# thenoobychocobo/gpt2-image-captioning

Measured on AMD Instinct MI355X. Metric: training images/sec + greedy captions/sec, GPT2-small+CLIP-B/32 at 1/2/4/8 GPU, higher is better.
Workload: dtype bf16

## Files before the change

gpt2-image-captioning_amd/csrc/gemm.hip:

```cpp
#include <cstdlib>

#include "gemm_tile.h"
#include "gemm_launch.h"

namespace icap {

template <typename TI>
__device__ __forceinline__ uint4 ln_chunk(const uint4 a, float mean, float rs, const float* g, const float* bt);
template <>
__device__ __forceinline__ uint4 ln_chunk<bf16_t>(const uint4 a, float mean, float rs, const float* g, const float* bt) {
  const uint32_t w[4] = {a.x, a.y, a.z, a.w};
  uint32_t o[4];
#pragma unroll
  for (int q = 0; q < 4; ++q) {
    const float v0 = (__uint_as_float(w[q] << 16) - mean) * rs * g[2 * q] + bt[2 * q];
    const float v1 = (__uint_as_float(w[q] & 0xffff0000u) - mean) * rs * g[2 * q + 1] + bt[2 * q + 1];
    o[q] = f2bf2(v0, v1);
  }
  return make_uint4(o[0], o[1], o[2], o[3]);
}
template <>
__device__ __forceinline__ uint4 ln_chunk<float>(const uint4 a, float mean, float rs, const float* g, const float* bt) {
  return make_uint4(__float_as_uint((__uint_as_float(a.x) - mean) * rs * g[0] + bt[0]),
                    __float_as_uint((__uint_as_float(a.y) - mean) * rs * g[1] + bt[1]),
// ... 359 lines not shown

static int gemm_acquire() { return diag_env("ICAP_FUSED_ACQUIRE", 0) == 1 ? 1 : 0; }
static int gemm_diag() { return diag_env("ICAP_GEMM_DIAG", 0) & 3; }

typedef int (*TileLauncher)(const GemmPlan&, const icap_gemm_args&, int, hipStream_t);
static TileLauncher tile_launcher(const GemmPlan& pl, const icap_gemm_args& p) {
  switch (pl.variant) {
    case V_ROLES_KOUT: return launch_tile_roles_kout;
    case V_ROLES: return launch_tile_roles;
    case V_ROLES160: return launch_tile_roles160;
    case V_ROLES96: return launch_tile_roles96;
    case V_ROLES192: return launch_tile_roles192;
    case V_R256: return launch_tile_r256;
    case V_W192: case V_W192_RING: return launch_tile_w192;
    case V_KOUT_DB: case V_KOUT_S3: return launch_tile_kout;
    case V_DB: case V_S3: case V_S4: case V_N12: case V_N13: case V_RING:
      if (pl.actk >= ACT_LNS) return launch_tile_ln;
      if (pl.actk >= ACT_FWD) return launch_tile_act;
      return p.in_dtype == ICAP_BF16 ? launch_tile_bf16 : p.in_dtype == ICAP_FP8_MX ? launch_tile_mx : launch_tile_f32;
  }
  return nullptr;
}

extern "C" const char* icap_gemm_kernel_name(const icap_gemm_args* a) {
  if (a == nullptr) return nullptr;
  GemmPlan pl;
  if (gemm_plan(*a, pl, device_cus(), plan_diag()) != ICAP_OK) return nullptr;
  return gemm_plan_kernel_name(*a, pl);
}

extern "C" int icap_gemm_plan_info(const icap_gemm_args* a, int32_t* splits, int32_t* fused) {
  ICAP_REQUIRE(a != nullptr && splits != nullptr && fused != nullptr, "icap_gemm_plan_info: null pointer");
  GemmPlan pl;
  const int rc = gemm_plan(*a, pl, device_cus(), plan_diag());
  if (rc != ICAP_OK) return rc;
  *splits = pl.skinny || pl.g256 || pl.g8p ? 1 : pl.splits;
  *fused = pl.fused ? 1 : 0;
  return ICAP_OK;
}

static bool group_force128() {
  const char* e = std::getenv("ICAP_GROUP128");
  return e != nullptr && std::atoi(e) == 1;
}

extern "C" int icap_gemm_group(const icap_gemm_args* a, int32_t n, void* stream) {
  ICAP_REQUIRE(a != nullptr && n >= 1 && n <= ICAP_GEMM_GROUP_MAX, "icap_gemm_group: 1 ... 8 products");
  static_assert(ICAP_GEMM_GROUP_MAX == GROUP_MAX, "the group's planner and its kernel argument hold the same count");
  GemmGroup g;
  g.n = 0;
  g.swap = 0;
  g.tstart[0] = 0;
  int64_t Ms[ICAP_GEMM_GROUP_MAX], Ns[ICAP_GEMM_GROUP_MAX];
  for (int i = 0; i < n; ++i) {
    const icap_gemm_args& p = a[i];
    icap_gemm_args q = p;
    q.split_k = 1;
    q.path = 0;
    if (const int rc = gemm_validate(q); rc != ICAP_OK) return rc;
    ICAP_REQUIRE(p.trans_ab && p.in_dtype == ICAP_BF16 && p.c_dtype == ICAP_F32,
                 "icap_gemm_group: K-outer (trans_ab) bf16 products with an fp32 C");
    ICAP_REQUIRE(p.act == ICAP_ACT_NONE && p.dact == ICAP_ACT_NONE && !p.bias && !p.resid && !p.aux && !p.ln_gamma &&
                     !p.ln_wsum && !p.ln_stats_in && !p.ln_stats_out && p.drop_p == 0.f && !p.m_dev,
                 "icap_gemm_group: plain products only (alpha, beta; no epilogue operands)");
    if (p.M == 0 || p.N == 0) continue;
    ICAP_REQUIRE(p.K > 0, "icap_gemm_group: K must be positive");
    const int k = g.n;
    g.a[k] = p;
    g.a[k].split_k = 1;
    g.a[k].tickets = nullptr;
    g.nk[k] = (int)((p.K + 63) / 64) | (gemm_diag() << 28);
    Ms[k] = p.M, Ns[k] = p.N;
    ++g.n;
  }
  if (g.n == 0) return ICAP_OK;
  const int cus = (int)device_cus();
  const GroupPlan gp = gemm_group_plan(Ms, Ns, g.n, cus, group_force128());
  ICAP_REQUIRE(gp.total < (1ll << 30), "icap_gemm_group: too many tiles");
  for (int k = 0; k < g.n; ++k) {
    if (gp.big && ((gp.swap >> k) & 1)) {
      icap_gemm_args& p = g.a[k];
      std::swap(p.A, p.B);
      std::swap(p.lda, p.ldb);
      std::swap(p.M, p.N);
    }
    g.tiles_n[k] = gp.tiles_n[k];
    g.tstart[k + 1] = g.tstart[k] + gp.tiles_m[k] * gp.tiles_n[k];
  }
  g.swap = gp.big ? gp.swap : 0u;
  launch_group_kout(g, cus, gp.big, reinterpret_cast<hipStream_t>(stream));
  return check_launch("icap_gemm_group");
}

extern "C" int icap_gemm(const icap_gemm_args* a, void* stream) {
  ICAP_REQUIRE(a != nullptr, "icap_gemm: null args");
  if (a->M == 0 || a->N == 0) return ICAP_OK;
  GemmPlan pl;
  const int prc = gemm_plan(*a, pl, device_cus(), plan_diag());
  if (prc != ICAP_OK) return prc;
  icap_gemm_args pk = *a;
  if (!pl.fused) pk.tickets = nullptr;
  const icap_gemm_args& p = pk;
  hipStream_t s = reinterpret_cast<hipStream_t>(stream);
  const uint32_t thr = pl.thr;
  const float inv_keep = pl.inv_keep;
  if (pl.skinny) {
    const dim3 sgrid(pl.grid_x, pl.grid_y), sblock(pl.block_x);
#define ICAP_SK(TI, TC, NT, U) hipLaunchKernelGGL((gemm_skinny_kernel<TI, TC, NT, 2, U>), sgrid, sblock, 0, s, p, thr, inv_keep)
#define ICAP_SKINNY_BF(TC)                                                                 \
  switch (pl.nt * 100 + pl.sku) {                                                          \
    case 103: ICAP_SK(bf16_t, TC, 1, 3); break;                                            \
    case 104: ICAP_SK(bf16_t, TC, 1, 4); break;                                            \
    case 106: ICAP_SK(bf16_t, TC, 1, 6); break;                                            \
    case 112: ICAP_SK(bf16_t, TC, 1, 12); break;                                           \
    case 203: ICAP_SK(bf16_t, TC, 2, 3); break;                                            \
    case 204: ICAP_SK(bf16_t, TC, 2, 4); break;                                            \
    case 206: ICAP_SK(bf16_t, TC, 2, 6); break;                                            \
    case 303: ICAP_SK(bf16_t, TC, 3, 3); break;                                            \
    case 304: ICAP_SK(bf16_t, TC, 3, 4); break;                                            \
    case 306: ICAP_SK(bf16_t, TC, 3, 6); break;                                            \
    case 403: ICAP_SK(bf16_t, TC, 4, 3); break;                                            \
    case 404: ICAP_SK(bf16_t, TC, 4, 4); break;                                            \
    default: ICAP_SK(bf16_t, TC, 4, 6); break;                                             \
  }
#define ICAP_SKINNY_F32(TC)                                                                \
  switch (pl.nt) {                                                                         \
    case 1: ICAP_SK(float, TC, 1, 6); break;                                               \
    case 2: ICAP_SK(float, TC, 2, 6); break;                                               \
    case 3: ICAP_SK(float, TC, 3, 6); break;                                               \
    default: ICAP_SK(float, TC, 4, 6); break;                                              \
  }
    if (p.in_dtype == ICAP_BF16) {
      if (p.c_dtype == ICAP_BF16) { ICAP_SKINNY_BF(bf16_t) } else { ICAP_SKINNY_BF(float) }
    } else {
      if (p.c_dtype == ICAP_BF16) { ICAP_SKINNY_F32(bf16_t) } else { ICAP_SKINNY_F32(float) }
    }
#undef ICAP_SKINNY_BF
#undef ICAP_SKINNY_F32
#undef ICAP_SK
    return check_launch("icap_gemm(skinny)");
  }
  if (pl.g256) return gemm256_launch(p, thr, inv_keep, s);
  if (pl.g8p) return gemm8p_launch(pl, p, s);
  const int sp = pl.splits;
  const int skew = gemm_plan_skew(p, pl, plan_diag());
  const int nks = pl.nk_split | (skew << 20) | (gemm_diag() << 28) | (gemm_acquire() << 30);
  const dim3 rgrid((unsigned)((p.M * (p.N / 4) + 255) / 256));
  const TileLauncher launch = tile_launcher(pl, p);
  if (launch == nullptr) return gemm_no_instantiation(pl);
  if (const int rc = launch(pl, p, nks, s); rc != ICAP_OK) return rc;
  if (sp > 1 && !pl.fused) {
    if (p.c_dtype == ICAP_BF16)
      hipLaunchKernelGGL((gemm_splitk_reduce<bf16_t>), rgrid, dim3(256), 0, s, p, sp, thr, inv_keep);
    else
      hipLaunchKernelGGL((gemm_splitk_reduce<float>), rgrid, dim3(256), 0, s, p, sp, thr, inv_keep);
  }
  return check_launch("icap_gemm");
}
```

gpt2-image-captioning_amd/csrc/gemm256.hip:

```cpp
#include "gemm_common.h"

namespace icap {
namespace g256 {
constexpr int BM = 256, BN = 256;
constexpr int HT = 128 * GROWB;
constexpr int TB = 4 * HT;
constexpr int ELD = 68;
constexpr int EW = 64 * ELD * 4;
constexpr int SMEM = (2 * TB > 8 * EW) ? 2 * TB : 8 * EW;
typedef uint32_t u32x4_t __attribute__((ext_vector_type(4)));
}

#define G256_RD(dst, addr, off) asm volatile("ds_read_b128 %0, %1 offset:" #off : "=v"(dst) : "v"(addr))

template <typename TC>
__global__ __launch_bounds__(512, 1) void gemm256_kernel(icap_gemm_args p, int tiles_n, uint32_t drop_thresh,
                                                        float inv_keep) {
  using namespace g256;
  __shared__ __attribute__((aligned(16))) char smem[SMEM];
  const int tid = threadIdx.x, lane = tid & 63;
  const int wave = __builtin_amdgcn_readfirstlane(tid >> 6);
  const int wr = wave >> 2, wc = wave & 3;
  const int fr = lane & 15, fg = lane >> 4;
  const int G = gridDim.x, bid = blockIdx.x;
  const int xcd = bid & 7, q8 = G >> 3, r8 = G & 7;
  const int wg = (xcd < r8 ? xcd * (q8 + 1) : r8 * (q8 + 1) + (xcd - r8) * q8) + (bid >> 3);
  const int tm = wg / tiles_n, tn = wg - tm * tiles_n;
  const int64_t M = p.M, N = p.N, K = p.K;
  const int64_t m0 = (int64_t)tm * BM, n0 = (int64_t)tn * BN;
  const int64_t mr = M - m0 < BM ? M - m0 : BM, nr = N - n0 < BN ? N - n0 : BN;
  const int nk = (int)((K + 63) / 64);
  const bf16_t* Ag = reinterpret_cast<const bf16_t*>(p.A);
  const bf16_t* Bg = reinterpret_cast<const bf16_t*>(p.B);
  const __amdgpu_buffer_rsrc_t ra = make_rsrc_u(Ag + m0 * p.lda, (uint64_t)((mr - 1) * p.lda + K) * 2);
  const __amdgpu_buffer_rsrc_t rb = make_rsrc_u(Bg + n0 * p.ldb, (uint64_t)((nr - 1) * p.ldb + K) * 2);

  const int c = (lane & 7) ^ (lane >> 3);
  uint32_t voff[4][2];
#pragma unroll
  for (int h = 0; h < 4; ++h)
#pragma unroll
    for (int i = 0; i < 2; ++i) {
      const int lr = (i * 8 + wave) * 8 + (lane >> 3);
      int trow;
      if (h == 0) trow = (lr & 63) + (lr >> 6) * 128;
      else if (h == 3) trow = (lr & 63) + (lr >> 6) * 128 + 64;
      else if (h == 1) trow = (lr >> 5) * 64 + (lr & 31);
      else trow = (lr >> 5) * 64 + 32 + (lr & 31);
      const int64_t ld = (h == 0 || h == 3) ? p.lda : p.ldb;
      voff[h][i] = (uint32_t)((trow * ld + c * 8) * 2);
// ... 183 lines not shown
```

gpt2-image-captioning_amd/csrc/gemm8p.hip:

```cpp
#include <utility>

#include "gemm_common.h"
#include "gemm_plan.h"

namespace icap {
namespace g8p {
constexpr int BM = 256;
constexpr int HTA = 128 * GROWB;
typedef uint32_t u32x4_t __attribute__((ext_vector_type(4)));
template <int BN>
struct Geo {
  static constexpr int WCN = BN / 4;
  static constexpr int QN = WCN / 2;
  static constexpr int NJ = QN / 16;
  static constexpr int HTB = (BN / 2) * GROWB;
  static constexpr int TB = 2 * HTA + 2 * HTB;
  static constexpr int BPW = BN / 128;
  static constexpr int ELD = WCN + 4;
  static constexpr int EW = 64 * ELD * 4;
  static constexpr int NBUF = BN == 128 ? 3 : 2;
  static constexpr int SMEM = (NBUF * TB > 8 * EW) ? NBUF * TB : 8 * EW;
  static constexpr int LPR = WCN / 8;
  static constexpr int RPI = 64 / LPR;
};
}

// ... 9 lines not shown

#define G8P_RD(dst, addr, off) asm volatile("ds_read_b128 %0, %1 offset:" #off : "=v"(dst) : "v"(addr))

template <typename TC, int BN, int ACT>
__global__ __launch_bounds__(512, 1) void gemm8p_kernel(icap_gemm_args p, int tiles_n, uint32_t drop_thresh,
                                                       float inv_keep) {
  using namespace g8p;
  using G = Geo<BN>;
  constexpr int AK = ACT & 0xFF;
  constexpr int LNX = ACT >> 8;
  constexpr int NJ = G::NJ, WCN = G::WCN, QN = G::QN, BPW = G::BPW, TB = G::TB, HTB = G::HTB, NBUF = G::NBUF;
  constexpr int LA = NBUF - 1;
  __shared__ __attribute__((aligned(16))) char smem[G::SMEM + (LNX == 2 ? 8 * BM : 0)];
  const int tid = threadIdx.x, lane = tid & 63;
  const int wave = __builtin_amdgcn_readfirstlane(tid >> 6);
  const int wr = wave >> 2, wc = wave & 3;
  const int fr = lane & 15, fg = lane >> 4;
  const int64_t M = p.M, N = p.N, K = p.K;
  const int64_t Mv = p.m_dev && (int64_t)*p.m_dev < M ? (int64_t)*p.m_dev : M;
  const int bid = blockIdx.x;
  const int tiles_mv = (int)((Mv + BM - 1) / BM);
  const int nwg = tiles_mv * tiles_n;
  if (bid >= nwg) return;
  const int xcd = bid & 7, q8 = nwg >> 3, r8 = nwg & 7;
  const int wg = (xcd < r8 ? xcd * (q8 + 1) : r8 * (q8 + 1) + (xcd - r8) * q8) + (bid >> 3);
  const int tm = wg / tiles_n, tn = wg - tm * tiles_n;
  const int64_t m0 = (int64_t)tm * BM, n0 = (int64_t)tn * BN;
  G8P_STAMP(1);
  const int64_t mr = Mv - m0 < BM ? Mv - m0 : BM, nr = N - n0 < BN ? N - n0 : BN;
  const int nk = (int)((K + 63) / 64);
  const bf16_t* Ag = reinterpret_cast<const bf16_t*>(p.A);
  const bf16_t* Bg = reinterpret_cast<const bf16_t*>(p.B);
  const __amdgpu_buffer_rsrc_t ra = make_rsrc_u(Ag + m0 * p.lda, (uint64_t)((mr - 1) * p.lda + K) * 2);
  const __amdgpu_buffer_rsrc_t rb = make_rsrc_u(Bg + n0 * p.ldb, (uint64_t)((nr - 1) * p.ldb + K) * 2);

  const int c = (lane & 7) ^ (lane >> 3);
  uint32_t voa[2][2], vob[2][BPW];
#pragma unroll
  for (int i = 0; i < 2; ++i) {
    const int lr = (i * 8 + wave) * 8 + (lane >> 3);
    const int trow = (lr & 63) + (lr >> 6) * 128;
    voa[0][i] = (uint32_t)((trow * p.lda + c * 8) * 2);
    voa[1][i] = (uint32_t)(((trow + 64) * p.lda + c * 8) * 2);
  }
#pragma unroll
  for (int i = 0; i < BPW; ++i) {
    const int lr = (i * 8 + wave) * 8 + (lane >> 3);
    const int trow = (lr / QN) * WCN + (lr % QN);
    vob[0][i] = (uint32_t)((trow * p.ldb + c * 8) * 2);
// ... 294 lines not shown
```

gpt2-image-captioning_amd/csrc/gemm_plan.cpp:

```cpp
#include "gemm_plan.h"

#include <cstdio>

namespace icap {

PlanDiag plan_diag() {
  PlanDiag d;
  d.var_heavy = diag_env("ICAP_VAR_HEAVY", d.var_heavy);
  d.var_act = diag_env("ICAP_VAR_ACT", d.var_act);
  d.var_light = diag_env("ICAP_VAR_LIGHT", d.var_light);
  d.fused_s = diag_env("ICAP_FUSED_S", d.fused_s);
  d.fused_nst = diag_env("ICAP_FUSED_NST", d.fused_nst);
  if (const int v = diag_env("ICAP_FUSED_MINK", 0); v >= 2) d.fused_mink = v;
  d.kskew = diag_env("ICAP_KSKEW", d.kskew);
  d.kout_fused = diag_env("ICAP_KOUT_FUSED", 0) == 1;
  d.spec_act = diag_env("ICAP_SPEC_ACT", 1) != 0;
  d.force_tile = diag_env("ICAP_FORCE_TILE", d.force_tile);
  d.w192r = diag_env("ICAP_W192R", d.w192r);
  return d;
}

static bool al16(const void* ptr) { return (reinterpret_cast<uintptr_t>(ptr) & 15) == 0; }
static int64_t cdiv(int64_t a, int64_t b) { return (a + b - 1) / b; }
static bool plain(const icap_gemm_args& p) { return p.act == ICAP_ACT_NONE && p.dact == ICAP_ACT_NONE; }

int gemm_validate(const icap_gemm_args& p) {
  ICAP_REQUIRE(p.M >= 0 && p.N >= 0 && p.K >= 0, "icap_gemm: negative size");
  ICAP_REQUIRE(p.path == 0 || p.path == 1 || (p.path >= 3 && p.path <= 12), "icap_gemm: path must be 0, 1 or 3 ... 12");
  ICAP_REQUIRE(p.A && p.B && p.C, "icap_gemm: null operand");
  ICAP_REQUIRE(p.in_dtype == ICAP_F32 || p.in_dtype == ICAP_BF16 || p.in_dtype == ICAP_FP8_MX,
               "icap_gemm: bad in_dtype");
  ICAP_REQUIRE(p.c_dtype == ICAP_F32 || p.c_dtype == ICAP_BF16, "icap_gemm: bad c_dtype");
  const bool mx = p.in_dtype == ICAP_FP8_MX;
  if (mx) {
    ICAP_REQUIRE(p.K % 128 == 0 && p.lda % 16 == 0 && p.ldb % 16 == 0,
                 "icap_gemm: FP8_MX needs K % 128 == 0 and lda, ldb multiples of 16");
    ICAP_REQUIRE(p.a_scale && p.b_scale && al16(p.a_scale) && al16(p.b_scale),
                 "icap_gemm: FP8_MX needs 16-byte aligned a_scale / b_scale");
    ICAP_REQUIRE(!p.trans_ab && !p.ln_gamma && p.path != 3, "icap_gemm: FP8_MX takes no trans_ab / ln / path 3");
    ICAP_REQUIRE((p.K / 32) * ((p.M + 63) / 64) * 64 < 0x7fffffffll && (p.K / 32) * ((p.N + 63) / 64) * 64 < 0x7fffffffll,
                 "icap_gemm: FP8_MX scale arrays must stay below 2 GiB");
// ... 332 lines not shown
    pl.nk_split = (int)c.nk;
    return ICAP_OK;
  }
  int rc;
  if ((rc = plan_skinny(c, pl)) != PASS) return rc;
  if ((rc = plan_g256(c, pl)) != PASS) return rc;
  if ((rc = plan_g8p(c, pl)) != PASS) return rc;
  if ((rc = plan_roles_kout(c, pl)) != PASS) return rc;
  TileSplit ts;
  if ((rc = plan_tile_split(c, ts)) != ICAP_OK) return rc;
  if ((rc = plan_roles(c, pl)) != PASS) return rc;
  if ((rc = plan_r256(c, ts, pl)) != PASS) return rc;
  if ((rc = plan_w192(c, ts, pl)) != PASS) return rc;
  return plan_tile128(c, ts, pl);
}

int gemm_plan_skew(const icap_gemm_args& p, const GemmPlan& pl, const PlanDiag& diag) {
  const TileVariantInfo* t = tile_variant(pl.variant);
  if (t == nullptr || t->natural_k()) return 0;
  if (p.path == 1 || p.path >= 6 || p.in_dtype == ICAP_FP8_MX || pl.nk_split > 64) return 0;
  return diag.kskew > 0 && diag.kskew < 256 ? diag.kskew : 0;
}

const char* gemm_plan_kernel_name(const icap_gemm_args& a, const GemmPlan& pl) {
  static thread_local char buf[160];
  const char* ti = a.in_dtype == ICAP_BF16 ? "unsigned short" : a.in_dtype == ICAP_FP8_MX ? "icap::fp8_t" : "float";
  const char* tc = a.c_dtype == ICAP_BF16 ? "unsigned short" : "float";
  if (pl.g256) {
    snprintf(buf, sizeof buf, "icap::gemm256_kernel<%s>", tc);
  } else if (pl.g8p) {
    snprintf(buf, sizeof buf, "icap::gemm8p_kernel<%s, %d, %d>", tc, pl.g8p, pl.actk);
  } else if (pl.skinny) {
    snprintf(buf, sizeof buf, "icap::gemm_skinny_kernel<%s, %s, %d, 2, %d>", ti, tc, pl.nt, pl.sku);
  } else if (const TileVariantInfo* t = tile_variant(pl.variant)) {
    snprintf(buf, sizeof buf, "icap::gemm_kernel<%s, %s, %d, %d, %d, %d, %d, %d, %s, %d%s>", ti, tc, t->nst, t->minb, t->wm,
             t->wn, t->tm, t->tn, t->kout ? "true" : "false", pl.actk, t->roles ? ", true" : "");
  } else {
    return nullptr;
  }
  return buf;
}

int gemm_no_instantiation(const GemmPlan& pl) {
  set_error("icap_gemm: no instantiation of " + (pl.g8p ? "the 8-phase kernel of width " + std::to_string(pl.g8p)
                                                         : "tile variant " + std::to_string(pl.variant)) +
            " with epilogue kind " + std::to_string(pl.actk) + " for these dtypes");
// ... 23 lines not shown
```

gpt2-image-captioning_amd/csrc/gemm_plan.h:

```cpp
#pragma once
#include "gemm_consts.h"
#include "host_common.h"

namespace icap {


struct EpiCaps {
  unsigned fwd = 0, bwd = 0;
  bool ln_producer = false;
  bool ln_consumer = false;
  unsigned ln_fwd = 0;
  bool ln_any = false;
  bool f32_c_plain = true;
};
constexpr unsigned A_(int act) { return 1u << act; }
constexpr unsigned A_GN = A_(ICAP_ACT_GELU_NEW), A_QG = A_(ICAP_ACT_QUICK_GELU), A_RELU = A_(ICAP_ACT_RELU),
                   A_ERF = A_(ICAP_ACT_GELU_ERF);
constexpr unsigned IN_F32 = 1u << ICAP_F32, IN_BF16 = 1u << ICAP_BF16, IN_MX = 1u << ICAP_FP8_MX;

enum TileVariant : int {
  V_DB = 0,
  V_S3 = 4,
  V_S4 = 5,
  V_N12 = 12,
// ... 82 lines not shown
  bool g256 = false;
  int g8p = 0;
  int nt = 1;
  int sku = 3;
  int variant = V_DB;
  int splits = 1, nk_split = 0, tiles_n = 0;
  bool fused = false;
  int actk = ACT_ANY;
  unsigned grid_x = 1, grid_y = 1, block_x = 1;
  uint32_t thr = 0;
  float inv_keep = 1.f;
};

struct PlanDiag {
  int var_heavy = V_S3, var_act = V_S3, var_light = V_S3;
  int fused_s = 0;
  int fused_nst = 0;
  int fused_mink = 24;
  int kskew = 1;
  bool kout_fused = false;
  bool spec_act = true;
  int force_tile = -1;
  int w192r = 4;
};
PlanDiag plan_diag();

int gemm_validate(const icap_gemm_args& p);
int gemm_plan(const icap_gemm_args& p, GemmPlan& pl, int cus, const PlanDiag& diag = PlanDiag());
int gemm_plan_skew(const icap_gemm_args& p, const GemmPlan& pl, const PlanDiag& diag = PlanDiag());
const char* gemm_plan_kernel_name(const icap_gemm_args& a, const GemmPlan& pl);
int gemm_no_instantiation(const GemmPlan& pl);

constexpr int GROUP_MAX = 8, GROUP_BM = 128, GROUP_BN_BIG = 256, GROUP_SWAP_N = 4;
struct GroupPlan {
  bool big = false;
  unsigned swap = 0;
  int tiles_m[GROUP_MAX] = {}, tiles_n[GROUP_MAX] = {};
  int64_t total = 0;
};
GroupPlan gemm_group_plan(const int64_t* M, const int64_t* N, int n, int cus, bool force128);

}
```

gpt2-image-captioning_amd/csrc/gemm_tile.h:

```cpp
#pragma once
#include "gemm_common.h"

#ifdef ICAP_STAMPS
#define ICAP_STAMP(i, v)                                                                                         \
  do {                                                                                                         \
    if (p.diag_stamps && threadIdx.x == 0) p.diag_stamps[(int64_t)blockIdx.x * 8 + (i)] = (uint64_t)(v);       \
  } while (0)
#define ICAP_NOW() __builtin_amdgcn_s_memrealtime()
#else
#define ICAP_STAMP(i, v) do {} while (0)
#define ICAP_NOW() 0ull
#endif

namespace icap {

__device__ __forceinline__ int kout_swz(int r) { return ((r & 3) << 2) | ((r >> 2) & 3); }
template <int ROWB = 256>
__device__ __forceinline__ int kout_off(int r, int ch) { return r * ROWB + ((ch ^ kout_swz(r)) << 4); }
typedef short kv4s_t __attribute__((ext_vector_type(4)));
typedef __attribute__((address_space(3))) kv4s_t* kout_lds_ptr;
template <int ROWB = 256>
__device__ __forceinline__ uint4 kout_frag(const char* img, int r0, int c0, int lane) {
  const int g = lane >> 4, q = (lane >> 2) & 3, pp = lane & 3;
  const int ch = (c0 >> 3) + (pp >> 1), half = (pp & 1) * 8;
// ... 49 lines not shown
  constexpr int NW = WM * WN;
  constexpr int BM = 16 * WM * TM, BN = 16 * WN * TN;
  constexpr int STB = (BM + BN) * GROWB;
  constexpr int EPR = (NST >= 2 && (16 * TM) % 32 == 0) ? 32 : 16;
  constexpr int ELD = 16 * TN + 4;
  static_assert(NW * EPR * ELD * 4 <= NST * STB, "epilogue staging must fit the stage buffers");
  static_assert(BM % (8 * NW) == 0 && BN % (8 * NW) == 0, "each wave stages whole 8-row DMA pieces");
  constexpr int APW = BM / (8 * NW), BPW = BN / (8 * NW);
  __shared__ __attribute__((aligned(16))) char smem[NST * STB + (LNX == 2 ? 8 * BM : 0)];
  constexpr int ES = sizeof(TI);
  constexpr int EPC = 16 / ES;
  constexpr int BKE = GROWB / ES;

  int tid = threadIdx.x;
  if constexpr (ROLES) asm volatile("" : "+v"(tid));
  const int lane = tid & 63;
  const int wave = tid >> 6;
  const int wm = wave / WN, wn = wave - wm * WN;

  const int64_t M = p.M, N = p.N, K = p.K;
  const int tiles_mv = p.m_dev ? (int)((Mv + BM - 1) / BM) : tiles_m;
  const int nwg = tiles_mv * tiles_n * splits;
  if (bid >= nwg) return;
  const int xcd = bid & 7, q = nwg >> 3, r = nwg & 7;
  const int wgid = (xcd < r ? xcd * (q + 1) : r * (q + 1) + (xcd - r) * q) + (bid >> 3);
  const int tiles = tiles_mv * tiles_n;
  const int split = wgid / tiles, tile = wgid - split * tiles;
  const int tm = tile / tiles_n, tn = tile - tm * tiles_n;
  const int64_t m0 = (int64_t)tm * BM, n0 = (int64_t)tn * BN;
  if (m0 >= Mv) return;
  ICAP_STAMP(1, ICAP_NOW());
  const char* Ab = reinterpret_cast<const char*>(p.A) + (KOUT ? m0 : m0 * p.lda) * ES;
  const char* Bb = reinterpret_cast<const char*>(p.B) + (KOUT ? n0 : n0 * p.ldb) * ES;
  const int64_t mrows = Mv - m0 < BM ? Mv - m0 : BM;
  const int64_t nrows = N - n0 < BN ? N - n0 : BN;
  const int diag = (nk_split >> 28) & 3;
  const bool acq = (nk_split >> 30) & 1;
  const __amdgpu_buffer_rsrc_t ra_rsrc = make_rsrc(
      Ab, (diag & 1) ? 0 : (uint64_t)(KOUT ? (K - 1) * p.lda + ((mrows + 7) & ~7ll) : (mrows - 1) * p.lda + K) * ES);
  const __amdgpu_buffer_rsrc_t rb_rsrc = make_rsrc(
      Bb, (diag & 2) ? 0 : (uint64_t)(KOUT ? (K - 1) * p.ldb + ((nrows + 7) & ~7ll) : (nrows - 1) * p.ldb + K) * ES);
  const int lrow = lane >> 3;
  const int lchunk = ((lane & 7) ^ lrow) * EPC;
  uint32_t a_off[APW], b_off[BPW];
  if constexpr (KOUT) {
    const int krow = lane >> 4;
#pragma unroll
    for (int i = 0; i < APW; ++i) {
      const int row = (wave * APW + i) * 4 + krow;
      a_off[i] = (uint32_t)(row * p.lda + (((lane & 15) ^ kout_swz(row)) << 3)) * ES;
    }
// ... 821 lines not shown
```

gpt2-image-captioning_amd/icap/_lib.py:

```python

from __future__ import annotations

import ctypes as C
import os

import torch

_HERE = os.path.dirname(os.path.abspath(__file__))
LIB_PATH = os.environ.get("ICAP_LIB") or os.path.join(_HERE, "libicap_hip.so")

F32, BF16, FP8_MX = 0, 1, 2
ACT_NONE, ACT_GELU_NEW, ACT_RELU, ACT_QUICK_GELU, ACT_TANH, ACT_GELU_ERF = 0, 1, 2, 3, 4, 5
AGG_MEAN, AGG_MAX, AGG_SUM_NORM = 0, 1, 2

vp = C.c_void_p
i32, i64, u64, f32, sz = C.c_int32, C.c_int64, C.c_uint64, C.c_float, C.c_size_t
pi32 = C.POINTER(C.c_int32)
pi64 = C.POINTER(C.c_int64)


class GemmArgs(C.Structure):
    _fields_ = [
        ("M", i64), ("N", i64), ("K", i64),
        ("in_dtype", i32), ("c_dtype", i32),
# ... 102 lines not shown
        ("hs", i32), ("vs", i32),
        ("restart_interval", i32),
        ("mcus_x", i32), ("mcus_y", i32),
        ("nseg", i32),
        ("blocks", i32),
        ("dc_tab", i32 * 3), ("ac_tab", i32 * 3),
        ("quant", (C.c_uint16 * 64) * 3),
        ("huff", JpegHuff * 4),
    ]


class JpegSegment(C.Structure):
    _fields_ = [("offset", i64), ("length", i64), ("first_mcu", i32), ("mcu_count", i32)]


SIGNATURES = {
    "icap_last_error": (C.c_char_p, []),
    "icap_version": (C.c_int, []),
    "icap_device_arch_ok": (C.c_int, []),
    "icap_gemm": (C.c_int, [C.POINTER(GemmArgs), vp]),
    "icap_gemm_group": (C.c_int, [C.POINTER(GemmArgs), C.c_int32, vp]),
    "icap_gemm_kernel_name": (C.c_char_p, [C.POINTER(GemmArgs)]),
    "icap_gemm_plan_info": (C.c_int, [C.POINTER(GemmArgs), vp, vp]),
    "icap_mx_scale_bytes": (sz, [i64, i64]),
    "icap_quantize_mx": (C.c_int, [i32, i64, i64, vp, i64, vp, i64, vp, vp, vp]),
    "icap_layernorm_fwd": (C.c_int, [i32, i64, i64, vp, i64, vp, vp, f32, vp, i64, vp, vp, vp, vp, vp]),
    "icap_layernorm_bwd_workspace_bytes": (sz, [i64, i64]),
    "icap_layernorm_bwd": (C.c_int, [i32, i64, i64, vp, i64, vp, vp, vp, vp, i64, vp, i64, vp, i64, vp,
                                     f32, u64, u64, vp, vp, vp, vp, vp, vp, i32, vp]),
    "icap_ln_param_reduce_batch": (C.c_int, [i32, C.POINTER(LnParamItem), vp]),
    "icap_attention_fwd": (C.c_int, [C.POINTER(AttnArgs), vp]),
    "icap_attention_bwd": (C.c_int, [C.POINTER(AttnArgs), vp]),
    "icap_attention_decode": (C.c_int, [i32, i32, i32, i32, i32, vp, i64, vp, i64, f32, vp]),
    "icap_attention_decode_anc": (C.c_int, [i32, i32, i32, i32, i32, vp, i64, vp, vp, i64, f32, vp]),
    "icap_beam_workspace_bytes": (C.c_size_t, [i32, i32, i32, i32]),
    "icap_beam_layout": (C.c_int, [i32, i32, i32, i32, vp]),
    "icap_beam_init": (C.c_int, [C.POINTER(BeamArgs), i32, vp]),
    "icap_beam_rowtop": (C.c_int, [i32, i64, i64, vp, i64, i32, vp, vp, vp, vp, vp]),
    "icap_beam_update": (C.c_int, [C.POINTER(BeamArgs), i32, i32, vp]),
    "icap_beam_finalize": (C.c_int, [C.POINTER(BeamArgs), vp, vp, vp]),
    "icap_gpt2_embed": (C.c_int, [i32, i32, i32, i32, i32, vp, i64, vp, vp, vp, vp, f32, u64, u64, vp, vp, vp, vp]),
    "icap_embedding_scatter_add": (C.c_int, [i32, i32, i32, i32, i32, vp, vp, vp, vp]),
    "icap_caption_prep": (C.c_int, [i32, i32, i32, vp, vp, vp, vp, vp, vp, vp, vp]),
    "icap_caption_pack": (C.c_int, [i32, i32, i32, vp, vp, vp, vp, vp, vp, vp, vp, vp, vp, vp]),
    "icap_rows_unpack": (C.c_int, [i32, i32, i32, i32, vp, vp, vp, vp, i64, vp]),
    "icap_cross_entropy_workspace_bytes": (sz, [i64]),
# ... 112 lines not shown
```

gpt2-image-captioning_amd/icap/ops.py:

```python

from __future__ import annotations

import contextlib
import ctypes as C
import os
import gc
from typing import Optional, Tuple

import torch

from . import _lib as L
from ._lib import AdamWArgs, AttnArgs, GemmArgs, call

Tensor = torch.Tensor


def dtype_code(t: torch.dtype) -> int:
    if t == torch.float32:
        return L.F32
    if t == torch.bfloat16:
        return L.BF16
    raise L.IcapError(f"unsupported storage dtype {t} (float32 or bfloat16)")


# ... 93 lines not shown
def quantize_mx(x: Tensor, out: Optional[MXTensor] = None, rows: Optional[int] = None,
                rows_dev: Optional[Tensor] = None) -> MXTensor:
    R = x.shape[0] if rows is None else rows
    K = x.shape[1]
    if out is None:
        out = MXTensor.empty(R, K, x.device)
    if out.R != R or out.K != K:
        raise L.IcapError("quantize_mx: output shape mismatch")
    call("icap_quantize_mx", dtype_code(x.dtype), R, K, x.data_ptr(), _ld(x), out.q.data_ptr(), _ld(out.q),
         out.scale.data_ptr(), _p(rows_dev), _stream())
    return out


def gemm(A: Tensor, B: Tensor, out: Tensor, *, bias: Optional[Tensor] = None, act: int = L.ACT_NONE,
         aux: Optional[Tensor] = None, dact: int = L.ACT_NONE, dact_src: Optional[Tensor] = None,
         resid: Optional[Tensor] = None, alpha: float = 1.0, beta: float = 0.0, drop: Dropout = NO_DROP,
         M: Optional[int] = None, N: Optional[int] = None, K: Optional[int] = None,
         alg_flops: Optional[float] = None, split_k: int = 0, m_dev: Optional[Tensor] = None,
         trans_ab: bool = False, ln: Optional[tuple] = None, workspace: Optional[Tensor] = None,
         tile_only: bool = False, g256: bool = False, g8p: int = 0, r256: bool = False, w192: bool = False,
         roles: int = 0, m_hint: Optional[int] = None,
         ln_fold: Optional[tuple] = None, ln_stats_out: Optional[Tensor] = None,
         ln_stats_in: Optional[Tensor] = None, ln_rows_out: Optional[tuple] = None,
         diag_stamps: Optional[Tensor] = None) -> Tensor:
    mx = isinstance(A, MXTensor)
    if mx != isinstance(B, MXTensor):
        raise L.IcapError("gemm: A and B must both be MXTensor (fp8 MX) or both plain tensors")
    if trans_ab:
        M = A.shape[1] if M is None else M
        K = A.shape[0] if K is None else K
        N = B.shape[1] if N is None else N
    else:
        M = A.shape[0] if M is None else M
        K = A.shape[1] if K is None else K
        N = B.shape[0] if N is None else N
    a = GemmArgs()
    a.trans_ab = 1 if trans_ab else 0
    a.M, a.N, a.K = M, N, K
    a.c_dtype = dtype_code(out.dtype)
    if mx:
        if M != A.R or N != B.R or K != A.K or K != B.K:
            raise L.IcapError("gemm: MX operands are whole matrices (M, N, K must equal their shapes)")
        a.in_dtype = L.FP8_MX
        a.A, a.lda = A.q.data_ptr(), _ld(A.q)
        a.B, a.ldb = B.q.data_ptr(), _ld(B.q)
        a.a_scale, a.b_scale = A.scale.data_ptr(), B.scale.data_ptr()
    else:
# ... 4 lines not shown
        a.B, a.ldb = B.data_ptr(), _ld(B)
    a.C, a.ldc = out.data_ptr(), _ld(out)
    a.alpha, a.beta = alpha, beta
    a.bias = _p(bias)
    a.act = act
    if aux is not None:
        a.aux, a.ldaux = aux.data_ptr(), _ld(aux)
    a.dact = dact
    if dact_src is not None:
        a.dact_src, a.ld_dact = dact_src.data_ptr(), _ld(dact_src)
    if resid is not None:
        a.resid, a.ldr = resid.data_ptr(), _ld(resid)
    a.drop_p, a.seed, a.offset, a.seed_ptr = drop.p, drop.seed, drop.offset, drop.ptr
    ws = gemm_workspace(A.device, torch.cuda.current_stream(A.device) if A.is_cuda else None) \
        if workspace is None else workspace
    a.workspace, a.workspace_bytes, a.split_k = ws.data_ptr(), ws.numel() * 4, split_k
    tk = _gemm_tickets.get(ws.data_ptr())
    if tk is not None and FUSED_SPLIT_K:
        a.tickets, a.tickets_len = tk.data_ptr(), tk.numel()
    a.m_dev = _p(m_dev)
    a.m_hint = int(m_hint) if (m_hint is not None and m_dev is not None) else 0
    a.path = (1 if tile_only else 3 if g256 else 4 if g8p == 128 else 5 if g8p == 256 else 6 if r256 else
              7 if w192 else 8 if roles == 256 else 9 if roles == 96 else 10 if roles == 192 else
              11 if roles == 1 else 12 if roles == 160 else 0)
    if ln is not None:
        a.ln_gamma, a.ln_beta, a.ln_eps = ln[0].data_ptr(), ln[1].data_ptr(), float(ln[2])
    if ln_fold is not None:
        a.ln_wsum, a.ln_eps = ln_fold[0].data_ptr(), float(ln_fold[1])
    if ln_stats_out is not None:
        a.ln_stats_out = ln_stats_out.data_ptr()
    if ln_stats_in is not None:
        a.ln_stats_in = ln_stats_in.data_ptr()
    if ln_rows_out is not None:
        a.ln_mean_out, a.ln_rstd_out = ln_rows_out[0].data_ptr(), ln_rows_out[1].data_ptr()
    if diag_stamps is not None:
        a.diag_stamps = diag_stamps.data_ptr()
    if GEMM_TIMER is None:
        call("icap_gemm", C.byref(a), _stream())
    else:
        name = L.load().icap_gemm_kernel_name(C.byref(a))
        key = (name.decode() if name else "?",
               f"{M}x{N}x{K} act{act} dact{dact} drop{int(drop.p > 0)} res{int(resid is not None)} "
               f"aux{int(aux is not None)} beta{beta:g}{' m_dev' if m_dev is not None else ''}"
               f"{' kout' if trans_ab else ''}{' ln' if ln is not None else ''}{' lnfold' if ln_fold is not None else ''}"
               f"{' lnS' if ln_stats_out is not None else ''}{' lnF' if ln_stats_in is not None else ''}")
        GEMM_TIMER.launch(key, 2.0 * M * N * K if alg_flops is None else alg_flops,
                          lambda: call("icap_gemm", C.byref(a), _stream()))
# ... 755 lines not shown
```

include/icap.h:

```cpp
#ifndef ICAP_H
#define ICAP_H

#include <stddef.h>
#include <stdint.h>

#ifdef __cplusplus
extern "C" {
#endif

enum { ICAP_F32 = 0, ICAP_BF16 = 1, ICAP_FP8_MX = 2 };
enum {
  ICAP_ACT_NONE = 0,
  ICAP_ACT_GELU_NEW = 1,
  ICAP_ACT_RELU = 2,
  ICAP_ACT_QUICK_GELU = 3,
  ICAP_ACT_TANH = 4,
  ICAP_ACT_GELU_ERF = 5
};
enum { ICAP_OK = 0, ICAP_ERR_ARG = 1, ICAP_ERR_LAUNCH = 2 };

const char* icap_last_error(void);
int icap_version(void);
int icap_device_arch_ok(void);

// ... 10 lines not shown
  void* aux; int64_t ldaux;
  int32_t dact;
  const void* dact_src; int64_t ld_dact;
  const void* resid; int64_t ldr;
  float drop_p; uint64_t seed; uint64_t offset;
  const uint64_t* seed_ptr;
  void* workspace; int64_t workspace_bytes; int32_t split_k;
  const int32_t* m_dev;
  int32_t trans_ab;
  const float* ln_gamma; const float* ln_beta; float ln_eps;
  int32_t path;
  const uint8_t* a_scale; const uint8_t* b_scale;
  int64_t m_hint;
  int32_t* tickets; int64_t tickets_len;
  const float* ln_wsum;
  float* ln_stats_out; const float* ln_stats_in; float* ln_mean_out; float* ln_rstd_out;
  uint64_t* diag_stamps;
} icap_gemm_args;
size_t icap_mx_scale_bytes(int64_t R, int64_t K);
int icap_quantize_mx(int32_t dtype, int64_t R, int64_t K, const void* x, int64_t ldx, void* q, int64_t ldq,
                     void* scales, const int32_t* rows_dev, void* stream);
const char* icap_gemm_kernel_name(const icap_gemm_args* a);
int icap_gemm_plan_info(const icap_gemm_args* a, int32_t* splits, int32_t* fused);
int icap_gemm(const icap_gemm_args* a, void* stream);
int icap_gemm_group(const icap_gemm_args* a, int32_t n, void* stream);

int icap_layernorm_fwd(int32_t dtype, int64_t rows, int64_t D, const void* x, int64_t ldx,
                       const float* gamma, const float* beta, float eps, void* y, int64_t ldy,
                       float* mean, float* rstd, const int32_t* y_rowmap, const int32_t* rows_dev,
                       void* stream);
size_t icap_layernorm_bwd_workspace_bytes(int64_t rows, int64_t D);
int icap_layernorm_bwd(int32_t dtype, int64_t rows, int64_t D, const void* x, int64_t ldx,
                       const float* gamma, const float* mean, const float* rstd,
                       const void* dy, int64_t lddy, const void* dres, int64_t lddres,
                       void* dx, int64_t lddx, void* dx_drop, float drop_p, uint64_t seed,
                       uint64_t offset, const uint64_t* seed_ptr, float* dgamma, float* dbeta,
                       void* workspace, const int32_t* dy_rowmap, const int32_t* rows_dev,
                       int32_t param_overwrite, void* stream);
#define ICAP_LN_PARAM_BATCH_MAX 16
typedef struct icap_ln_param_item {
  const void* workspace; int64_t rows; int64_t D; float* dgamma; float* dbeta; int32_t overwrite;
} icap_ln_param_item;
int icap_ln_param_reduce_batch(int32_t n, const icap_ln_param_item* items, void* stream);

typedef struct {
  int32_t dtype;
// ... 204 lines not shown
```

Measured before the change: 15020.

## Add grouped (banded) tile rasterization for GEMM kernels chosen by a byte-traffic model

Adds a banded tile-to-workgroup mapping in which each band of gm row tiles is walked column-major, applied after the XCD chunking in the tile, 256 and 8p GEMM kernels. The planner picks gm from a model of how many distinct A and B bytes the concurrently resident tiles per XCD touch, and applies it only to selected shape classes (wide and vocab by default). The aim is better L2 reuse of operand tiles within each XCD. It adds a small index computation per workgroup and carries the raster value in the path field, with environment overrides and a host-side check tool.

```diff
diff --git a/gpt2-image-captioning_amd/csrc/gemm.hip b/gpt2-image-captioning_amd/csrc/gemm.hip
--- a/gpt2-image-captioning_amd/csrc/gemm.hip
+++ b/gpt2-image-captioning_amd/csrc/gemm.hip
@@ -405,20 +405,50 @@
   return nullptr;
 }
 
-extern "C" const char* icap_gemm_kernel_name(const icap_gemm_args* a) {
-  if (a == nullptr) return nullptr;
+static icap_gemm_args split_path(const icap_gemm_args& a, int& raster) {
+  icap_gemm_args q = a;
+  raster = a.path >> 8;
+  q.path = a.path & 0xFF;
+  return q;
+}
+#define ICAP_REQUIRE_RASTER(r) \
+  ICAP_REQUIRE((r) >= 0, "icap_gemm: raster (path >> 8) must be 0 (automatic), 1 (row-major) or a band height >= 2")
+
+extern "C" const char* icap_gemm_kernel_name(const icap_gemm_args* a0) {
+  if (a0 == nullptr) return nullptr;
+  int raster;
+  const icap_gemm_args q = split_path(*a0, raster);
+  const icap_gemm_args* a = &q;
+  if (raster < 0) return nullptr;
   GemmPlan pl;
   if (gemm_plan(*a, pl, device_cus(), plan_diag()) != ICAP_OK) return nullptr;
   return gemm_plan_kernel_name(*a, pl);
 }
 
-extern "C" int icap_gemm_plan_info(const icap_gemm_args* a, int32_t* splits, int32_t* fused) {
-  ICAP_REQUIRE(a != nullptr && splits != nullptr && fused != nullptr, "icap_gemm_plan_info: null pointer");
+extern "C" int icap_gemm_plan_info(const icap_gemm_args* a0, int32_t* splits, int32_t* fused) {
+  ICAP_REQUIRE(a0 != nullptr && splits != nullptr && fused != nullptr, "icap_gemm_plan_info: null pointer");
+  int raster;
+  const icap_gemm_args q = split_path(*a0, raster);
+  const icap_gemm_args* a = &q;
+  ICAP_REQUIRE_RASTER(raster);
   GemmPlan pl;
   const int rc = gemm_plan(*a, pl, device_cus(), plan_diag());
   if (rc != ICAP_OK) return rc;
   *splits = pl.skinny || pl.g256 || pl.g8p ? 1 : pl.splits;
   *fused = pl.fused ? 1 : 0;
+  return ICAP_OK;
+}
+
+extern "C" int icap_gemm_raster(const icap_gemm_args* a0, int32_t* gm) {
+  ICAP_REQUIRE(a0 != nullptr && gm != nullptr, "icap_gemm_raster: null pointer");
+  int raster;
+  const icap_gemm_args q = split_path(*a0, raster);
+  const icap_gemm_args* a = &q;
+  ICAP_REQUIRE_RASTER(raster);
+  GemmPlan pl;
+  const int rc = gemm_plan(*a, pl, device_cus(), plan_diag());
+  if (rc != ICAP_OK) return rc;
+  *gm = gemm_plan_raster(*a, pl, (int)device_cus(), raster, plan_diag());
   return ICAP_OK;
 }
 
@@ -452,6 +482,7 @@
     g.a[k] = p;
     g.a[k].split_k = 1;
     g.a[k].tickets = nullptr;
+    g.a[k].path = 1;
     g.nk[k] = (int)((p.K + 63) / 64) | (gemm_diag() << 28);
     Ms[k] = p.M, Ns[k] = p.N;
     ++g.n;
@@ -475,14 +506,19 @@
   return check_launch("icap_gemm_group");
 }
 
-extern "C" int icap_gemm(const icap_gemm_args* a, void* stream) {
-  ICAP_REQUIRE(a != nullptr, "icap_gemm: null args");
+extern "C" int icap_gemm(const icap_gemm_args* a0, void* stream) {
+  ICAP_REQUIRE(a0 != nullptr, "icap_gemm: null args");
+  int raster;
+  const icap_gemm_args q = split_path(*a0, raster);
+  const icap_gemm_args* a = &q;
+  ICAP_REQUIRE_RASTER(raster);
   if (a->M == 0 || a->N == 0) return ICAP_OK;
   GemmPlan pl;
   const int prc = gemm_plan(*a, pl, device_cus(), plan_diag());
   if (prc != ICAP_OK) return prc;
   icap_gemm_args pk = *a;
   if (!pl.fused) pk.tickets = nullptr;
+  pk.path = gemm_plan_raster(*a, pl, (int)device_cus(), raster, plan_diag());
   const icap_gemm_args& p = pk;
   hipStream_t s = reinterpret_cast<hipStream_t>(stream);
   const uint32_t thr = pl.thr;
@@ -526,7 +562,7 @@
   if (pl.g256) return gemm256_launch(p, thr, inv_keep, s);
   if (pl.g8p) return gemm8p_launch(pl, p, s);
   const int sp = pl.splits;
-  const int skew = gemm_plan_skew(p, pl, plan_diag());
+  const int skew = gemm_plan_skew(*a, pl, plan_diag());
   const int nks = pl.nk_split | (skew << 20) | (gemm_diag() << 28) | (gemm_acquire() << 30);
   const dim3 rgrid((unsigned)((p.M * (p.N / 4) + 255) / 256));
   const TileLauncher launch = tile_launcher(pl, p);
diff --git a/gpt2-image-captioning_amd/csrc/gemm256.hip b/gpt2-image-captioning_amd/csrc/gemm256.hip
--- a/gpt2-image-captioning_amd/csrc/gemm256.hip
+++ b/gpt2-image-captioning_amd/csrc/gemm256.hip
@@ -1,4 +1,5 @@
 #include "gemm_common.h"
+#include "gemm_raster.h"
 
 namespace icap {
 namespace g256 {
@@ -23,9 +24,8 @@
   const int wr = wave >> 2, wc = wave & 3;
   const int fr = lane & 15, fg = lane >> 4;
   const int G = gridDim.x, bid = blockIdx.x;
-  const int xcd = bid & 7, q8 = G >> 3, r8 = G & 7;
-  const int wg = (xcd < r8 ? xcd * (q8 + 1) : r8 * (q8 + 1) + (xcd - r8) * q8) + (bid >> 3);
-  const int tm = wg / tiles_n, tn = wg - tm * tiles_n;
+  const RasterTile rt = raster_tile(xcd_chunk(bid, G), G / tiles_n, tiles_n, p.path);
+  const int tm = rt.tm, tn = rt.tn;
   const int64_t M = p.M, N = p.N, K = p.K;
   const int64_t m0 = (int64_t)tm * BM, n0 = (int64_t)tn * BN;
   const int64_t mr = M - m0 < BM ? M - m0 : BM, nr = N - n0 < BN ? N - n0 : BN;
diff --git a/gpt2-image-captioning_amd/csrc/gemm8p.hip b/gpt2-image-captioning_amd/csrc/gemm8p.hip
--- a/gpt2-image-captioning_amd/csrc/gemm8p.hip
+++ b/gpt2-image-captioning_amd/csrc/gemm8p.hip
@@ -2,6 +2,7 @@
 
 #include "gemm_common.h"
 #include "gemm_plan.h"
+#include "gemm_raster.h"
 
 namespace icap {
 namespace g8p {
@@ -57,9 +58,8 @@
   const int tiles_mv = (int)((Mv + BM - 1) / BM);
   const int nwg = tiles_mv * tiles_n;
   if (bid >= nwg) return;
-  const int xcd = bid & 7, q8 = nwg >> 3, r8 = nwg & 7;
-  const int wg = (xcd < r8 ? xcd * (q8 + 1) : r8 * (q8 + 1) + (xcd - r8) * q8) + (bid >> 3);
-  const int tm = wg / tiles_n, tn = wg - tm * tiles_n;
+  const RasterTile rt = raster_tile(xcd_chunk(bid, nwg), tiles_mv, tiles_n, p.path);
+  const int tm = rt.tm, tn = rt.tn;
   const int64_t m0 = (int64_t)tm * BM, n0 = (int64_t)tn * BN;
   G8P_STAMP(1);
   const int64_t mr = Mv - m0 < BM ? Mv - m0 : BM, nr = N - n0 < BN ? N - n0 : BN;
diff --git a/gpt2-image-captioning_amd/csrc/gemm_plan.cpp b/gpt2-image-captioning_amd/csrc/gemm_plan.cpp
--- a/gpt2-image-captioning_amd/csrc/gemm_plan.cpp
+++ b/gpt2-image-captioning_amd/csrc/gemm_plan.cpp
@@ -17,6 +17,8 @@
   d.spec_act = diag_env("ICAP_SPEC_ACT", 1) != 0;
   d.force_tile = diag_env("ICAP_FORCE_TILE", d.force_tile);
   d.w192r = diag_env("ICAP_W192R", d.w192r);
+  d.raster_gm = diag_env("ICAP_RASTER_GM", d.raster_gm);
+  d.raster_classes = diag_env("ICAP_RASTER_CLASSES", d.raster_classes);
   return d;
 }
 
@@ -395,6 +397,46 @@
   return diag.kskew > 0 && diag.kskew < 256 ? diag.kskew : 0;
 }
 
+int64_t raster_model_bytes(int64_t tiles_m, int64_t tiles_n, int64_t q, int64_t gm, int64_t bm, int64_t bn, int64_t K,
+                           int64_t es) {
+  const int64_t g = gm < 1 ? 1 : gm > tiles_m ? tiles_m : gm;
+  const int64_t cq = cdiv(q, g), cols = cq < tiles_n ? cq : tiles_n;
+  const int64_t rq = g * cdiv(q, g * tiles_n), rows = rq < tiles_m ? rq : tiles_m;
+  return (rows * bm + cols * bn) * K * es;
+}
+constexpr int RASTER_KEPT = RC_WIDE | RC_VOCAB;
+int gemm_plan_raster(const icap_gemm_args& p, const GemmPlan& pl, int cus, int raster, const PlanDiag& diag) {
+  if (pl.skinny || p.M <= 0 || p.N <= 0) return 1;
+  const TileVariantInfo* t = tile_variant(pl.variant);
+  const bool ring8 = pl.g256 || pl.g8p;
+  if (!ring8 && t == nullptr) return 1;
+  const int64_t bm = ring8 ? 256 : t->bm(), bn = pl.g256 ? 256 : pl.g8p ? pl.g8p : t->bn();
+  const int64_t per_cu = ring8 ? 1 : t->minb;
+  const int64_t cap_m = cdiv(p.M, bm);
+  const int forced = raster >= 1 ? raster : diag.raster_gm >= 1 ? diag.raster_gm : 0;
+  if (forced) return (int)(forced < cap_m ? forced : cap_m);
+  if (p.in_dtype != ICAP_BF16 || p.trans_ab) return 1;
+  const int64_t m_plan = (p.m_dev && p.m_hint > 0 && p.m_hint < p.M) ? p.m_hint : p.M;
+  const int64_t tiles_m = cdiv(m_plan, bm), tiles_n = cdiv(p.N, bn), tiles = tiles_m * tiles_n;
+  const int cls = p.N <= 1024 ? RC_NARROW
+                  : (p.K > 1536 || p.dact != ICAP_ACT_NONE) ? RC_NONE
+                  : p.N >= 16384 ? RC_VOCAB
+                  : tiles <= cus * per_cu ? RC_ROUND : RC_WIDE;
+  if (!((diag.raster_classes >= 0 ? diag.raster_classes : RASTER_KEPT) & cls)) return 1;
+  const int64_t xcds = 8, conc = (cus / xcds > 0 ? cus / xcds : 1) * per_cu;
+  int64_t q = cdiv(tiles * (pl.splits > 1 ? pl.splits : 1), xcds);
+  if (q > conc) q = conc;
+  if (q > tiles) q = tiles;
+  const int64_t es = 2;
+  int64_t best = 1, best_bytes = raster_model_bytes(tiles_m, tiles_n, q, 1, bm, bn, p.K, es);
+  for (int64_t g = 2; g <= tiles_m && g <= q; ++g) {
+    if (tiles_m % g) continue;
+    const int64_t b = raster_model_bytes(tiles_m, tiles_n, q, g, bm, bn, p.K, es);
+    if (b < best_bytes) best = g, best_bytes = b;
+  }
+  return (int)best;
+}
+
 const char* gemm_plan_kernel_name(const icap_gemm_args& a, const GemmPlan& pl) {
   static thread_local char buf[160];
   const char* ti = a.in_dtype == ICAP_BF16 ? "unsigned short" : a.in_dtype == ICAP_FP8_MX ? "icap::fp8_t" : "float";
diff --git a/gpt2-image-captioning_amd/csrc/gemm_plan.h b/gpt2-image-captioning_amd/csrc/gemm_plan.h
--- a/gpt2-image-captioning_amd/csrc/gemm_plan.h
+++ b/gpt2-image-captioning_amd/csrc/gemm_plan.h
@@ -128,12 +128,24 @@
   bool spec_act = true;
   int force_tile = -1;
   int w192r = 4;
+  int raster_gm = 0;
+  int raster_classes = -1;
 };
 PlanDiag plan_diag();
 
 int gemm_validate(const icap_gemm_args& p);
 int gemm_plan(const icap_gemm_args& p, GemmPlan& pl, int cus, const PlanDiag& diag = PlanDiag());
 int gemm_plan_skew(const icap_gemm_args& p, const GemmPlan& pl, const PlanDiag& diag = PlanDiag());
+enum RasterClass : int {
+  RC_NONE = 0,
+  RC_WIDE = 1,
+  RC_ROUND = 2,
+  RC_VOCAB = 4,
+  RC_NARROW = 8,
+};
+int gemm_plan_raster(const icap_gemm_args& p, const GemmPlan& pl, int cus, int raster, const PlanDiag& diag = PlanDiag());
+int64_t raster_model_bytes(int64_t tiles_m, int64_t tiles_n, int64_t q, int64_t gm, int64_t bm, int64_t bn, int64_t K,
+                           int64_t es);
 const char* gemm_plan_kernel_name(const icap_gemm_args& a, const GemmPlan& pl);
 int gemm_no_instantiation(const GemmPlan& pl);
 
diff --git a/gpt2-image-captioning_amd/csrc/gemm_raster.h b/gpt2-image-captioning_amd/csrc/gemm_raster.h
--- /dev/null
+++ b/gpt2-image-captioning_amd/csrc/gemm_raster.h
@@ -0,0 +1,33 @@
+#pragma once
+
+#if defined(__HIPCC__)
+#define ICAP_RASTER_FN __host__ __device__ inline
+#else
+#define ICAP_RASTER_FN inline
+#endif
+
+namespace icap {
+
+constexpr int RASTER_XCDS = 8;
+
+ICAP_RASTER_FN int xcd_chunk(int bid, int live) {
+  const int xcd = bid & (RASTER_XCDS - 1), q = live / RASTER_XCDS, r = live & (RASTER_XCDS - 1);
+  return (xcd < r ? xcd * (q + 1) : r * (q + 1) + (xcd - r) * q) + bid / RASTER_XCDS;
+}
+
+struct RasterTile {
+  int tm, tn;
+};
+ICAP_RASTER_FN RasterTile raster_tile(int idx, int tiles_m, int tiles_n, int gm) {
+  if (gm <= 1) {
+    const int tm = idx / tiles_n;
+    return {tm, idx - tm * tiles_n};
+  }
+  const int per_band = gm * tiles_n;
+  const int band = idx / per_band, in = idx - band * per_band;
+  const int left = tiles_m - band * gm, rows = left < gm ? left : gm;
+  const int tn = in / rows;
+  return {band * gm + (in - tn * rows), tn};
+}
+
+}
diff --git a/gpt2-image-captioning_amd/csrc/gemm_tile.h b/gpt2-image-captioning_amd/csrc/gemm_tile.h
--- a/gpt2-image-captioning_amd/csrc/gemm_tile.h
+++ b/gpt2-image-captioning_amd/csrc/gemm_tile.h
@@ -1,5 +1,6 @@
 #pragma once
 #include "gemm_common.h"
+#include "gemm_raster.h"
 
 #ifdef ICAP_STAMPS
 #define ICAP_STAMP(i, v)                                                                                         \
@@ -95,11 +96,11 @@
   const int tiles_mv = p.m_dev ? (int)((Mv + BM - 1) / BM) : tiles_m;
   const int nwg = tiles_mv * tiles_n * splits;
   if (bid >= nwg) return;
-  const int xcd = bid & 7, q = nwg >> 3, r = nwg & 7;
-  const int wgid = (xcd < r ? xcd * (q + 1) : r * (q + 1) + (xcd - r) * q) + (bid >> 3);
+  const int wgid = xcd_chunk(bid, nwg);
   const int tiles = tiles_mv * tiles_n;
   const int split = wgid / tiles, tile = wgid - split * tiles;
-  const int tm = tile / tiles_n, tn = tile - tm * tiles_n;
+  const RasterTile rt = raster_tile(tile, tiles_mv, tiles_n, p.path);
+  const int tm = rt.tm, tn = rt.tn;
   const int64_t m0 = (int64_t)tm * BM, n0 = (int64_t)tn * BN;
   if (m0 >= Mv) return;
   ICAP_STAMP(1, ICAP_NOW());
diff --git a/gpt2-image-captioning_amd/csrc/raster_check.cpp b/gpt2-image-captioning_amd/csrc/raster_check.cpp
--- /dev/null
+++ b/gpt2-image-captioning_amd/csrc/raster_check.cpp
@@ -0,0 +1,125 @@
+#include <cstdio>
+#include <cstdlib>
+#include <cstring>
+#include <iostream>
+#include <sstream>
+#include <string>
+#include <vector>
+
+#include "gemm_plan.h"
+#include "gemm_raster.h"
+
+namespace icap {
+static std::string g_err;
+void set_error(const std::string& m) { g_err = m; }
+}
+using namespace icap;
+
+static void parent_map(int bid, int nwg, int tiles, int tiles_n, int& split, int& tm, int& tn) {
+  const int xcd = bid & 7, q = nwg >> 3, r = nwg & 7;
+  const int wgid = (xcd < r ? xcd * (q + 1) : r * (q + 1) + (xcd - r) * q) + (bid >> 3);
+  split = wgid / tiles;
+  const int tile = wgid - split * tiles;
+  tm = tile / tiles_n, tn = tile - tm * tiles_n;
+}
+
+static bool check_grid(int tiles_m, int tiles_n, long long& cases) {
+  const int tiles = tiles_m * tiles_n;
+  std::vector<unsigned char> seen;
+  for (int splits = 1; splits <= 4; ++splits) {
+    const int live = tiles * splits;
+    for (int gm = 1; gm <= tiles_m + 1; ++gm) {
+      seen.assign((size_t)live, 0);
+      for (int bid = 0; bid < live; ++bid) {
+        const int wg = xcd_chunk(bid, live);
+        if (wg < 0 || wg >= live) return std::fprintf(stderr, "chunk out of range\n"), false;
+        const int split = wg / tiles;
+        const RasterTile t = raster_tile(wg - split * tiles, tiles_m, tiles_n, gm);
+        if (t.tm < 0 || t.tm >= tiles_m || t.tn < 0 || t.tn >= tiles_n)
+          return std::fprintf(stderr, "%d x %d gm %d splits %d bid %d: tile (%d, %d) out of range\n", tiles_m, tiles_n, gm,
+                              splits, bid, t.tm, t.tn), false;
+        unsigned char& s = seen[((size_t)split * tiles_m + t.tm) * tiles_n + t.tn];
+        if (s) return std::fprintf(stderr, "%d x %d gm %d splits %d: tile (%d, %d, %d) twice\n", tiles_m, tiles_n, gm,
+                                   splits, split, t.tm, t.tn), false;
+        s = 1;
+        if (gm == 1) {
+          int ps, pm, pn;
+          parent_map(bid, live, tiles, tiles_n, ps, pm, pn);
+          if (ps != split || pm != t.tm || pn != t.tn)
+            return std::fprintf(stderr, "%d x %d splits %d bid %d: gm 1 is not the row-major map\n", tiles_m, tiles_n,
+                                splits, bid), false;
+        }
+      }
+      ++cases;
+    }
+  }
+  return true;
+}
+
+template <typename T>
+static T* fake(uintptr_t v) { return reinterpret_cast<T*>(v); }
+
+int main(int argc, char** argv) {
+  const std::string mode = argc > 1 ? argv[1] : "";
+  if (mode == "sweep") {
+    long long cases = 0;
+    for (int m = 1; m <= 40; ++m)
+      for (int n = 1; n <= 40; ++n)
+        if (!check_grid(m, n, cases)) return 1;
+    const int extra[3][2] = {{7, 197}, {50, 24}, {28, 24}};
+    for (const auto& e : extra)
+      if (!check_grid(e[0], e[1], cases)) return 1;
+    std::printf("ok %lld\n", cases);
+    return 0;
+  }
+  if (mode == "rect" && argc == 5) {
+    const int tiles_m = std::atoi(argv[2]), tiles_n = std::atoi(argv[3]), gm = std::atoi(argv[4]);
+    if (tiles_m < 1 || tiles_n < 1 || gm < 1) return 2;
+    const int live = tiles_m * tiles_n;
+    for (int x = 0; x < RASTER_XCDS; ++x) {
+      int lo_m = tiles_m, hi_m = -1, lo_n = tiles_n, hi_n = -1, count = 0;
+      for (int bid = x; bid < live; bid += RASTER_XCDS) {
+        const RasterTile t = raster_tile(xcd_chunk(bid, live), tiles_m, tiles_n, gm);
+        lo_m = t.tm < lo_m ? t.tm : lo_m, hi_m = t.tm > hi_m ? t.tm : hi_m;
+        lo_n = t.tn < lo_n ? t.tn : lo_n, hi_n = t.tn > hi_n ? t.tn : hi_n;
+        ++count;
+      }
+      std::printf("%d %d %d %d %d %d\n", x, lo_m, hi_m, lo_n, hi_n, count);
+    }
+    return 0;
+  }
+  if (mode == "plan") {
+    std::string line;
+    while (std::getline(std::cin, line)) {
+      std::istringstream in(line);
+      long long cus, M, N, K, m_hint;
+      int act, dact, aux, raster;
+      if (!(in >> cus >> M >> N >> K >> m_hint >> act >> dact >> aux >> raster)) continue;
+      icap_gemm_args a;
+      std::memset(&a, 0, sizeof a);
+      a.M = M, a.N = N, a.K = K;
+      a.in_dtype = a.c_dtype = ICAP_BF16;
+      a.A = a.B = a.C = fake<void>(1u << 20);
+      a.lda = a.ldb = K, a.ldc = N;
+      a.alpha = 1.f;
+      a.workspace = fake<void>(1u << 21), a.workspace_bytes = 1ll << 40;
+      a.tickets = fake<int32_t>(1u << 22), a.tickets_len = 1ll << 30;
+      a.act = act, a.dact = dact;
+      if (aux) a.aux = fake<void>(1u << 24), a.ldaux = N;
+      if (dact) a.dact_src = fake<void>(1u << 24), a.ld_dact = N;
+      if (m_hint > 0) a.m_dev = fake<const int32_t>(1u << 25), a.m_hint = m_hint;
+      GemmPlan pl;
+      if (gemm_plan(a, pl, (int)cus) != ICAP_OK) {
+        std::printf("error %s\n", g_err.c_str());
+        continue;
+      }
+      const TileVariantInfo* t = tile_variant(pl.variant);
+      const bool ring8 = pl.g256 || pl.g8p;
+      const int bm = pl.skinny ? 0 : ring8 ? 256 : t->bm(), bn = pl.skinny ? 0 : pl.g256 ? 256 : pl.g8p ? pl.g8p : t->bn();
+      std::printf("%d %d %d %s\n", gemm_plan_raster(a, pl, (int)cus, raster), bm, bn, gemm_plan_kernel_name(a, pl));
+    }
+    return 0;
+  }
+  std::fprintf(stderr, "usage: raster_check sweep | rect TM TN GM | plan < shapes\n");
+  return 2;
+}
diff --git a/gpt2-image-captioning_amd/icap/_lib.py b/gpt2-image-captioning_amd/icap/_lib.py
--- a/gpt2-image-captioning_amd/icap/_lib.py
+++ b/gpt2-image-captioning_amd/icap/_lib.py
@@ -148,6 +148,7 @@
     "icap_gemm_group": (C.c_int, [C.POINTER(GemmArgs), C.c_int32, vp]),
     "icap_gemm_kernel_name": (C.c_char_p, [C.POINTER(GemmArgs)]),
     "icap_gemm_plan_info": (C.c_int, [C.POINTER(GemmArgs), vp, vp]),
+    "icap_gemm_raster": (C.c_int, [C.POINTER(GemmArgs), vp]),
     "icap_mx_scale_bytes": (sz, [i64, i64]),
     "icap_quantize_mx": (C.c_int, [i32, i64, i64, vp, i64, vp, i64, vp, vp, vp]),
     "icap_layernorm_fwd": (C.c_int, [i32, i64, i64, vp, i64, vp, vp, f32, vp, i64, vp, vp, vp, vp, vp]),
diff --git a/gpt2-image-captioning_amd/icap/ops.py b/gpt2-image-captioning_amd/icap/ops.py
--- a/gpt2-image-captioning_amd/icap/ops.py
+++ b/gpt2-image-captioning_amd/icap/ops.py
@@ -139,7 +139,7 @@
          roles: int = 0, m_hint: Optional[int] = None,
          ln_fold: Optional[tuple] = None, ln_stats_out: Optional[Tensor] = None,
          ln_stats_in: Optional[Tensor] = None, ln_rows_out: Optional[tuple] = None,
-         diag_stamps: Optional[Tensor] = None) -> Tensor:
+         diag_stamps: Optional[Tensor] = None, raster: int = 0) -> Tensor:
     mx = isinstance(A, MXTensor)
     if mx != isinstance(B, MXTensor):
         raise L.IcapError("gemm: A and B must both be MXTensor (fp8 MX) or both plain tensors")
@@ -190,7 +190,7 @@
     a.m_hint = int(m_hint) if (m_hint is not None and m_dev is not None) else 0
     a.path = (1 if tile_only else 3 if g256 else 4 if g8p == 128 else 5 if g8p == 256 else 6 if r256 else
               7 if w192 else 8 if roles == 256 else 9 if roles == 96 else 10 if roles == 192 else
-              11 if roles == 1 else 12 if roles == 160 else 0)
+              11 if roles == 1 else 12 if roles == 160 else 0) | (raster << 8)
     if ln is not None:
         a.ln_gamma, a.ln_beta, a.ln_eps = ln[0].data_ptr(), ln[1].data_ptr(), float(ln[2])
     if ln_fold is not None:
diff --git a/include/icap.h b/include/icap.h
--- a/include/icap.h
+++ b/include/icap.h
@@ -56,6 +56,8 @@
                      void* scales, const int32_t* rows_dev, void* stream);
 const char* icap_gemm_kernel_name(const icap_gemm_args* a);
 int icap_gemm_plan_info(const icap_gemm_args* a, int32_t* splits, int32_t* fused);
+#define ICAP_GEMM_PATH(number, raster) ((int32_t)(number) | ((int32_t)(raster) << 8))
+int icap_gemm_raster(const icap_gemm_args* a, int32_t* gm);
 int icap_gemm(const icap_gemm_args* a, void* stream);
 int icap_gemm_group(const icap_gemm_args* a, int32_t n, void* stream);
 
```

Measured after the change: 15020. No clear change (-0.0%).
